# sloisel/MultiGridBarrierMPI.jl

Hardware: AMD Instinct MI355X
Metric: fem2d p-Laplace DoF/s per Newton step (higher is better)
Workload: dtype f64; 1 GPU; fem2d p-Laplace L=7 p=1 (n=57344 rows, N_L=49154 Newton unknowns), amgb main phase, tol=sqrt(eps); parallelism=single GPU

## Files before the change

include/mgb_hip.h:

```cpp
#ifndef MGB_HIP_H
#define MGB_HIP_H

#include <stdint.h>

#ifdef __cplusplus
extern "C" {
#endif

#define MGB_OK 0
#define MGB_E_ARG (-1)
#define MGB_E_HIP (-2)
#define MGB_E_NUMERIC (-3)
#define MGB_E_INTERNAL (-4)

typedef struct mgb_ctx_s* mgb_ctx;
typedef struct mgb_geo_s* mgb_geo;
typedef struct mgb_amg_s* mgb_amg;
typedef struct mgb_vec_s* mgb_vec;
typedef struct mgb_csr_s* mgb_csr;

const char* mgb_last_error(void);
int mgb_version(void);
int mgb_device_count(void);

// ... 116 lines not shown
int mgb_plan_prolongation(mgb_plan fine, mgb_plan coarse, int* rows, int* cols, int* nnz, int32_t* rowptr, int32_t* colidx,
                          double* vals);
int mgb_plan_sizes(mgb_plan p, int* N, int* nnz_lower, int* nnz_T, int* nnz_B);
int mgb_plan_pattern(mgb_plan p, int32_t* rowptr, int32_t* colidx);
int mgb_plan_eval_host(mgb_plan p, const double* Y , double* lower_vals);
int mgb_plan_shard(mgb_plan p, int S, int K, int rank, int world, int block, mgb_plan* out, int* r0, int* r1);
int mgb_plan_apply_B_host(mgb_plan p, const double* s , double* Bs );
int mgb_plan_apply_BT_host(mgb_plan p, const double* v , double* g );
int mgb_plan_chol_bench(mgb_plan p, const double* Y, int dim, int reps, double* seconds_per_factor,
                        double* seconds_per_solve, double* flops, double* front_doubles, double* residual);
typedef struct mgb_hostchol_s* mgb_hostchol;
int mgb_plan_hostchol_create(mgb_plan p, int dim, mgb_hostchol* out);
int mgb_hostchol_destroy(mgb_hostchol c);
int mgb_hostchol_info(mgb_hostchol c, int* n, int* threads, double* flops);
int mgb_hostchol_factor_solve(mgb_hostchol c, const double* lower_vals, const double* g, double* x);
int mgb_hostchol_partition(mgb_hostchol c, int world, int* split_world, int cap, int* nnodes, int* owner);
int mgb_hostchol_factor_solve_dist(mgb_hostchol c, int rank, int world, mgb_allreduce_fn fn, void* user,
                                   const double* lower_vals, const double* g, double* x);
int mgb_plan_hostchol_create_ranked(mgb_plan p, int dim, int K, int world, int block, mgb_hostchol* out);
int mgb_hostchol_rank_aligned(mgb_hostchol c, int world, int* aligned, int* top_values);
int mgb_hostchol_factor_solve_dist_local(mgb_hostchol c, int rank, int world, mgb_allreduce_fn fn, void* user,
                                         const double* local_lower_vals, const double* g, double* x);
int mgb_plan_chol_tree(mgb_plan p, int dim, int cap, int* nnodes, int* ns, int* nf, int* parent);
int mgb_chol_selftest(int nx, int ny, double* max_residual, double* flops, double* seconds);

#ifdef __cplusplus
}
#endif
#endif
```

multigridbarriermpi.jl_amd/_lib.py:

```python
from __future__ import annotations

import ctypes as C
import os

import numpy as np

_HERE = os.path.dirname(os.path.abspath(__file__))
LIB_PATH = os.path.join(_HERE, "lib", "libmgb_hip.so")

c_int_p = C.POINTER(C.c_int)
c_i32_p = C.POINTER(C.c_int32)
c_dbl_p = C.POINTER(C.c_double)
c_flt_p = C.POINTER(C.c_float)
c_ll_p = C.POINTER(C.c_longlong)
c_str_arr = C.POINTER(C.c_char_p)
H = C.c_void_p
ALLREDUCE_FN = C.CFUNCTYPE(C.c_int, C.c_void_p, C.c_void_p, C.c_longlong)


class MGBError(RuntimeError):
    def __init__(self, code, msg):
        super().__init__("mgb error %d: %s" % (code, msg))
        self.code = code

# ... 97 lines not shown
    "mgb_amg_sol_kernels": [H, c_dbl_p, c_dbl_p, c_ll_p],
    "mgb_amg_time_kernels": [H, C.c_int, C.c_int, C.c_int, c_dbl_p, c_dbl_p],
    "mgb_plan_create": [H, C.c_int, c_str_arr, C.c_int, c_str_arr, C.c_int, c_int_p, C.c_int, C.c_int,
                        C.POINTER(H)],
    "mgb_reduction_scratch_doubles": [C.c_int, C.c_int, c_ll_p],
    "mgb_plan_destroy": [H],
    "mgb_plan_sizes": [H, c_int_p, c_int_p, c_int_p, c_int_p],
    "mgb_plan_pattern": [H, c_i32_p, c_i32_p],
    "mgb_plan_eval_host": [H, c_dbl_p, c_dbl_p],
    "mgb_plan_shard": [H, C.c_int, C.c_int, C.c_int, C.c_int, C.c_int, C.POINTER(C.c_void_p), c_int_p, c_int_p],
    "mgb_plan_apply_B_host": [H, c_dbl_p, c_dbl_p],
    "mgb_plan_apply_BT_host": [H, c_dbl_p, c_dbl_p],
    "mgb_plan_chol_bench": [H, c_dbl_p, C.c_int, C.c_int, c_dbl_p, c_dbl_p, c_dbl_p, c_dbl_p, c_dbl_p],
    "mgb_plan_hostchol_create": [H, C.c_int, C.POINTER(H)],
    "mgb_hostchol_destroy": [H],
    "mgb_hostchol_info": [H, c_int_p, c_int_p, c_dbl_p],
    "mgb_hostchol_factor_solve": [H, c_dbl_p, c_dbl_p, c_dbl_p],
    "mgb_hostchol_partition": [H, C.c_int, c_int_p, C.c_int, c_int_p, c_int_p],
    "mgb_hostchol_factor_solve_dist": [H, C.c_int, C.c_int, ALLREDUCE_FN, C.c_void_p, c_dbl_p, c_dbl_p, c_dbl_p],
    "mgb_plan_hostchol_create_ranked": [H, C.c_int, C.c_int, C.c_int, C.c_int, C.POINTER(H)],
    "mgb_hostchol_rank_aligned": [H, C.c_int, c_int_p, c_int_p],
    "mgb_hostchol_factor_solve_dist_local": [H, C.c_int, C.c_int, ALLREDUCE_FN, C.c_void_p, c_dbl_p, c_dbl_p, c_dbl_p],
    "mgb_plan_chol_tree": [H, C.c_int, C.c_int, c_int_p, c_int_p, c_int_p, c_int_p],
    "mgb_chol_selftest": [C.c_int, C.c_int, c_dbl_p, c_dbl_p, c_dbl_p],
}
_SPECIAL = {"mgb_last_error": ([], C.c_char_p), "mgb_version": ([], C.c_int), "mgb_device_count": ([], C.c_int)}

_lib = None


def load():
    global _lib
    if _lib is not None:
        return _lib
    if not os.path.exists(LIB_PATH):
        raise ImportError("libmgb_hip.so not built: run `python -c 'import __graft_entry__ as g; g.build()'` "
                          "or multigridbarriermpi.jl_amd/csrc/build.sh (expected at %s)" % LIB_PATH)
    lib = C.CDLL(LIB_PATH)
    for name, args in PROTOTYPES.items():
        fn = getattr(lib, name)
        fn.argtypes = args
        fn.restype = C.c_int
    for name, (args, res) in _SPECIAL.items():
        fn = getattr(lib, name)
        fn.argtypes = args
        fn.restype = res
# ... 34 lines not shown
```

multigridbarriermpi.jl_amd/csrc/capi.cpp:

```cpp
#include "../../include/mgb_hip.h"

#include <chrono>
#include <cmath>
#include <cstdlib>
#include <string>
#include <thread>

#include "amg.hpp"

using namespace mgb;

struct mgb_ctx_s {
  Ctx ctx;
  explicit mgb_ctx_s(int dev) : ctx(dev) {}
};
struct mgb_geo_s {
  GeometryHost g;
};
struct mgb_vec_s {
  mgb_ctx_s* ctx;
  DevBuf<double> buf;
  int n;
};
struct mgb_csr_s {
// ... 1254 lines not shown
      const int rc = fn(user, ptr, count);
      if (rc != 0) throw InternalError("mgb: allreduce callback failed with code " + std::to_string(rc));
    };
    if (!c->ch.factor_solve_dist(local_lower_vals, x, part, rank, ar, true))
      throw NumericError("MfChol: matrix is not positive definite");
  });
}

int mgb_plan_chol_tree(mgb_plan p, int dim, int cap, int* nnodes, int* ns, int* nf, int* parent) {
  return guard([&] {
    need(p && nnodes, "chol_tree: bad arguments");
    MfChol ch;
    ch.analyze(p->plan.Apat, p->plan.coords.data(), dim);
    std::vector<int> a, b, c;
    ch.tree(a, b, c);
    *nnodes = (int)a.size();
    const int m = std::min<int>(cap, (int)a.size());
    if (ns) std::copy(a.begin(), a.begin() + m, ns);
    if (nf) std::copy(b.begin(), b.begin() + m, nf);
    if (parent) std::copy(c.begin(), c.begin() + m, parent);
  });
}

int mgb_chol_selftest(int nx, int ny, double* max_residual, double* flops, double* seconds) {
  return guard([&] {
    need(nx > 0 && ny > 0, "selftest: bad size");
    const int N = nx * ny;
    std::vector<Triplet> t;
    std::vector<double> coords((size_t)N * 2);
    for (int j = 0; j < ny; ++j)
      for (int i = 0; i < nx; ++i) {
        const int r = j * nx + i;
        coords[2 * r] = i;
        coords[2 * r + 1] = j;
        t.push_back({r, r, 6.0 + 1e-3 * ((r * 7919) % 13)});
        if (i > 0) t.push_back({r, r - 1, -1.0});
        if (j > 0) t.push_back({r, r - nx, -1.0});
        if (i > 0 && j > 0) t.push_back({r, r - nx - 1, -0.5});
      }
    Csr Lo = from_triplets(N, N, t);
    MfChol ch;
    ch.analyze(Lo, coords.data(), 2);
    const auto t0 = std::chrono::steady_clock::now();
    if (!ch.factor(Lo.vals.data())) throw NumericError("MfChol: selftest matrix not SPD");
    const double sec = std::chrono::duration<double>(std::chrono::steady_clock::now() - t0).count();
    std::vector<double> xs(N), b(N, 0.0);
// ... 18 lines not shown
```

multigridbarriermpi.jl_amd/csrc/gpuchol.hip:

```cpp
#include "gpuchol.hpp"

#include "amg.hpp"

#include <algorithm>
#include <array>
#include <cmath>
#include <cstdio>
#include <cstdlib>
#include <numeric>
#include <stdexcept>
#include <string>

namespace mgb {

namespace {

constexpr int PB = 32;
constexpr int LP = PB + 1;
constexpr int TS = 64;
constexpr int TB = 256;
constexpr int RT = 1024;

void ck(hipError_t e, const char* what) {
  if (e != hipSuccess) throw HipError(std::string("HIP error in gpuchol ") + what + ": " + hipGetErrorString(e));
// ... 1153 lines not shown
          for (int i = k0 + sl; i < k1; i += nsl) s = fma(F[(long long)ld * i + j], u[i], s);
        }
        if (nsl > 1) {
          red[tid] = s;
          __syncthreads();
          if (sl == 0)
            for (int q = 1; q < nsl; ++q) s += red[q * jw + jl];
        }
        if (sl == 0 && j < k0) u[j] -= s;
      }
      __syncthreads();
    }
    if (pp == npanel - 1) STAMP(5);
  }
  STAMP(6);
  for (int i = tid; i < ns; i += NT) {
    const double v = u[i];
    y[nd.first + i] = v;
    x[perm[nd.first + i]] = v;
  }
  STAMP(7);
}

__global__ __launch_bounds__(256) void schur_pack_kernel(const RootXchg* __restrict__ roots, const double* __restrict__ fronts,
                                                         double* __restrict__ xb) {
  const RootXchg r = roots[blockIdx.x];
  const double* F = fronts + r.off;
  for (int j = blockIdx.y; j < r.nb; j += gridDim.y) {
    double* dst = xb + r.xoff + (long long)j * (r.nb + 1) - (long long)j * (j - 1) / 2 - j;
    const double* col = F + (long long)r.ld * (r.ns + j) + r.ns;
    for (int i = j + threadIdx.x; i <= r.nb; i += blockDim.x) dst[i] = r.owned ? col[i] : 0.0;
  }
}

__global__ __launch_bounds__(256) void schur_unpack_kernel(const RootXchg* __restrict__ roots, const double* __restrict__ xb,
                                                           double* __restrict__ fronts) {
  const RootXchg r = roots[blockIdx.x];
  double* F = fronts + r.off;
  for (int j = blockIdx.y; j < r.nb; j += gridDim.y) {
    const double* src = xb + r.xoff + (long long)j * (r.nb + 1) - (long long)j * (j - 1) / 2 - j;
    double* col = F + (long long)r.ld * (r.ns + j) + r.ns;
    for (int i = j + threadIdx.x; i <= r.nb; i += blockDim.x) col[i] = src[i];
  }
}

__global__ __launch_bounds__(256) void vals_pack_kernel(int n, const int* __restrict__ idx, const double* __restrict__ vals,
// ... 50 lines not shown
};

const CholKnobs& GpuChol::knobs() {
  static const CholKnobs k = [] {
    auto on = [](const char* name) {
      const char* e = std::getenv(name);
      return !(e && e[0] == '0');
    };
    auto num = [](const char* name, int dflt) {
      const char* e = std::getenv(name);
      return e ? std::atoi(e) : dflt;
    };
    CholKnobs c;
    c.graph = on("MGB_CHOL_GRAPH");
    c.prof = std::getenv("MGB_CHOL_PROF") != nullptr;
    c.leaf = on("MGB_CHOL_LEAF");
    c.single = on("MGB_CHOL_SINGLE");
    c.step2 = on("MGB_CHOL_STEP2");
    c.wide = on("MGB_CHOL_WIDE");
    c.start_pivot = on("MGB_CHOL_START_PIVOT");
    c.step2_tiles = num("MGB_CHOL_STEP2_TILES", 224);
    c.dense_tiles = num("MGB_CHOL_DENSE_TILES", 512);
    c.bwd_split_nf = num("MGB_BWD_SPLIT_NF", 192);
    return c;
  }();
  return k;
}

namespace {

StepTile pivot_tile(const GNode& g, int t, int p) {
  StepTile st{};
  st.off = g.off;
  st.loff = g.loff + (long long)p * 2 * PB * PB;
  st.nf = g.nf;
  st.ns = g.ns;
  st.pad = t;
  return st;
}

int append_tiles(std::vector<StepTile>& out, const GNode& g, int t, int p, int k, bool column) {
  StepTile st = pivot_tile(g, t, p);
  const size_t n0 = out.size();
  if (column) {
    const int Tr = std::max(0, (g.nf + 1 - k - PB + TS - 1) / TS);
    for (int ti = 0; ti < Tr; ++ti) {
// ... 25 lines not shown
  u.a1 = g.a1;
  u.first = g.first;
  u.ti = s.ti;
  u.tj = s.tj;
  for (int sI = 0; sI < 2; ++sI) {
    u.boff[sI] = g.off;
    u.cld[sI] = 0;
    if (g.child[sI] >= 0) {
      const GNode& c = nodes[g.child[sI]];
      u.cld[sI] = c.nf + 1;
      u.boff[sI] = c.off + (long long)u.cld[sI] * c.ns + c.ns;
    }
  }
  return u;
}

}

int GpuChol::schedule(const std::vector<std::vector<int>>& heights, const std::vector<GNode>& nodes,
                      const std::vector<std::vector<StartJob>>& sjobs, const MfChol& sym, Jobs& jobs) {
  const CholKnobs& kn = knobs();
  std::vector<Launch> bwd;
  std::vector<StepTile> scratch;
  for (const std::vector<int>& mine : heights) {
    if (mine.empty()) continue;
    const int nofs = (int)jobs.lists.size(), ncnt = (int)mine.size();
    jobs.lists.insert(jobs.lists.end(), mine.begin(), mine.end());
    int max_ns = 0, max_nf = 0;
    bool childless = true, all_pivots = true;
    double start_bytes = 0;
    for (int t : mine) {
      const GNode& g = nodes[t];
      max_ns = std::max(max_ns, g.ns);
      max_nf = std::max(max_nf, g.nf);
      childless = childless && g.child[0] < 0 && g.child[1] < 0;
      all_pivots = all_pivots && g.ns >= 1;
      start_bytes += 0.5 * g.nf * g.nf * 8.0 + (double)sym.a_idx_[t].size() * 20.0;
      for (int c : g.child) {
        if (c < 0) continue;
        const double cnb = nodes[c].nf - nodes[c].ns;
        start_bytes += 0.5 * cnb * cnb * 8.0;
      }
    }
    const bool leaf = kn.leaf && max_nf <= 95 && max_ns <= 2 * PB && childless && all_pivots;
    const bool single = kn.single && max_ns <= PB && !childless && all_pivots;
    if (leaf) {
      const size_t lds = ((size_t)(max_nf + 1) * max_nf - (size_t)max_nf * (max_nf - 1) / 2) * sizeof(double);
// ... 68 lines not shown
      if (single) {
        const int sofs = (int)jobs.singles.size();
        for (int q = ofs; q < ofs + cnt; ++q) jobs.singles.push_back(single_tile(nodes, jobs.tiles[q]));
        const bool narrow = max_ns <= 8, dense = cnt > kn.dense_tiles;
        const Kind k = dense ? (narrow ? Kind::SingleDenseNarrow : Kind::SingleDense) : (narrow ? Kind::SingleNarrow : Kind::Single);
        chain_.push_back({k, sofs, cnt, TB, 0, 0, 0, false, KC_CHOL_SINGLE, start_bytes + bytes});
      } else {
        chain_.push_back({pair ? Kind::Step2 : Kind::Step, ofs, cnt, TB, pair ? (size_t)kStep2Lds : 0, p, npiv, false, KC_CHOL_STEP, bytes});
      }
      if (pair) ++p;
    }
    const bool split = max_nf > kn.bwd_split_nf;
    const int rofs = (int)jobs.rects.size();
    double rect_bytes = 0, tri_bytes = 0;
    for (int t : mine) {
      const GNode& g = nodes[t];
      const double nb = g.nf - g.ns;
      rect_bytes += nb * g.ns * 8.0 + nb * 12.0;
      tri_bytes += 0.5 * g.ns * g.ns * 8.0 + g.ns * 28.0;
      if (split && nb > 0)
        for (int ch = 0; ch * 64 < g.ns; ++ch) jobs.rects.push_back({t, ch});
    }
    const int nrect = (int)jobs.rects.size() - rofs, nt = max_nf > 384 ? 1024 : 256;
    std::vector<Launch> h;
    if (nrect) h.push_back({Kind::BwdRect, rofs, nrect, RT, (size_t)(max_nf + RT) * sizeof(double), 0, 0, false, KC_CHOL_BWD_RECT, rect_bytes});
    h.push_back({nt == 1024 ? Kind::Bwd1024 : Kind::Bwd256, nofs, ncnt, nt, (size_t)(max_nf + nt + PB) * sizeof(double), 0, 0, nrect > 0,
                 KC_CHOL_BWD, tri_bytes + (nrect ? 0.0 : rect_bytes)});
    bwd.insert(bwd.begin(), h.begin(), h.end());
  }
  const int first_bwd = (int)chain_.size();
  chain_.insert(chain_.end(), bwd.begin(), bwd.end());
  return first_bwd;
}

void GpuChol::build(const MfChol& sym, Ctx* ctx) {
  ctx_ = ctx;
  part_ = (ctx && ctx->world > 1) ? sym.partition(ctx->world) : CholPartition();
  if (!part_.split()) part_.owner.assign(sym.nodes_.size(), -1);
  const int my_rank = ctx ? ctx->rank : 0;
  n_ = sym.n_;
  nnodes_ = (int)sym.nodes_.size();
  flops_ = sym.flops_;
  std::vector<GNode> nodes(nnodes_);
  std::vector<int> bdry_all, ea_all, pinv, height(nnodes_, 0);
  long long off = 0, loff = 0;
  max_nf_ = 0;
  for (int t = 0; t < nnodes_; ++t) {
    const auto& nd = sym.nodes_[t];
    GNode& g = nodes[t];
    g.off = off;
    g.loff = loff;
    loff += (long long)((nd.ns + PB - 1) / PB) * 2 * PB * PB;
    g.nf = nd.nf();
    g.ns = nd.ns;
// ... 74 lines not shown
        j.a0 = (int)asrc.size();
        while (q < m && key(ord[q]) == (long long)ch * 65536 + rb) {
          const int pos = sym.a_pos_[t][ord[q]], col = pos / nf, row = pos % nf;
          if (row < col) throw InternalError("gpuchol: assembly entry above the diagonal");
          asrc.push_back(sym.a_idx_[t][ord[q]]);
          apos.push_back(ld * col + row);
          ++q;
        }
        j.a1 = (int)asrc.size();
        sjobs[t].push_back(j);
      }
    }
    if (q != m) throw InternalError("gpuchol: assembly entry outside the front");
    nodes[t].a0 = sjobs[t].empty() ? 0 : sjobs[t].front().a0;
    nodes[t].a1 = sjobs[t].empty() ? 0 : sjobs[t].back().a1;
  }
  std::vector<std::vector<int>> own(nheights_), top(nheights_);
  for (int t = 0; t < nnodes_; ++t) {
    if (!part_.split() || part_.owner[t] == my_rank) own[height[t]].push_back(t);
    else if (part_.owner[t] < 0) top[height[t]].push_back(t);
  }
  Jobs jobs;
  chain_.clear();
  own_bwd_ = schedule(own, nodes, sjobs, sym, jobs);
  top_fwd_ = (int)chain_.size();
  if (part_.split()) schedule(top, nodes, sjobs, sym, jobs);
  if ((size_t)(max_nf_ + RT + PB) * 8 > 150 * 1024) throw ArgError("gpuchol: front exceeds the LDS budget of the sweeps");
  d_nodes_ = upload(nodes);
  d_perm_ = upload(sym.perm_);
  d_bdry_ = upload(bdry_all);
  d_pinv_ = upload(pinv);
  d_asm_src_ = upload(asrc);
  d_asm_pos_ = upload(apos);
  d_lists_ = upload(jobs.lists);
  {
    std::vector<GNode> hn(jobs.lists.size()), rn(jobs.rects.size());
    for (size_t k = 0; k < jobs.lists.size(); ++k) hn[k] = nodes[jobs.lists[k]];
    for (size_t k = 0; k < jobs.rects.size(); ++k) rn[k] = nodes[jobs.rects[k].node];
    d_hnodes_ = upload(hn);
    d_rnodes_ = upload(rn);
  }
  d_start_ = upload(jobs.starts);
  d_tiles_ = upload(jobs.tiles);
  d_singles_ = upload(jobs.singles);
  d_rectjobs_ = upload(jobs.rects);
  if (part_.split()) {
    std::vector<RootXchg> roots;
    long long xoff = 0;
    for (int j = 0; j < part_.world; ++j) {
      const GNode& g = nodes[part_.roots[j]];
      RootXchg r{};
      r.off = g.off;
      r.xoff = xoff;
      r.ld = g.nf + 1;
      r.ns = g.ns;
      r.nb = g.nf - g.ns;
      r.owned = (j == my_rank) ? 1 : 0;
      xoff += (long long)r.nb * (r.nb + 3) / 2;
      max_root_nb_ = std::max(max_root_nb_, r.nb);
      roots.push_back(r);
    }
    xchg_doubles_ = xoff;
    nroots_ = (int)roots.size();
    d_roots_ = upload(roots);
    std::vector<int> own(n_, 0);
    for (int t = 0; t < nnodes_; ++t)
      if (part_.owner[t] == my_rank || (part_.owner[t] < 0 && my_rank == 0))
        for (int k = 0; k < nodes[t].ns; ++k) own[sym.perm_[nodes[t].first + k]] = 1;
// ... 32 lines not shown
  ck(hipMalloc((void**)&d_fail_, sizeof(int)), "hipMalloc flag");
  allocs_.push_back(d_fail_);
  ck(hipMemset(d_fail_, 0, sizeof(int)), "memset");
  if (knobs().prof) {
    const size_t nl = chain_.size();
    ck(hipMalloc((void**)&d_prof_, kProfSlots * nl * sizeof(long long)), "hipMalloc prof");
    allocs_.push_back(d_prof_);
    reset_stamps();
#ifdef MGB_PROF_PER_WG
    {
      long long* wg = nullptr;
      ck(hipMalloc((void**)&wg, nl * kProfMaxWg * 2 * sizeof(long long)), "hipMalloc wgprof");
      allocs_.push_back(wg);
      ck(hipMemset(wg, 0, nl * kProfMaxWg * 2 * sizeof(long long)), "memset wgprof");
      ck(hipMemcpyToSymbol(HIP_SYMBOL(g_wgprof), &wg, sizeof(wg)), "symbol wgprof");
      ck(hipMemcpyToSymbol(HIP_SYMBOL(g_prof_base), &d_prof_, sizeof(d_prof_)), "symbol prof base");
      d_wgprof_ = wg;
    }
#endif
  }
  ck(hipFuncSetAttribute((const void*)backward_kernel<256>, hipFuncAttributeMaxDynamicSharedMemorySize, 150 * 1024), "attr");
  ck(hipFuncSetAttribute((const void*)backward_kernel<1024>, hipFuncAttributeMaxDynamicSharedMemorySize, 150 * 1024), "attr");
  ck(hipFuncSetAttribute((const void*)backward_rect_kernel, hipFuncAttributeMaxDynamicSharedMemorySize, 150 * 1024), "attr");
  ck(hipFuncSetAttribute((const void*)front_leaf_kernel, hipFuncAttributeMaxDynamicSharedMemorySize, 100 * 1024), "attr");
  ck(hipFuncSetAttribute((const void*)front_step2_kernel, hipFuncAttributeMaxDynamicSharedMemorySize, kStep2Lds), "attr");
  ck(hipFuncSetAttribute((const void*)front_panel2_kernel, hipFuncAttributeMaxDynamicSharedMemorySize, kPanel2Lds), "attr");
  ck(hipFuncSetAttribute((const void*)front_update2_kernel, hipFuncAttributeMaxDynamicSharedMemorySize, kUpdate2Lds), "attr");
}

void GpuChol::factor_solve(hipStream_t st, double* d_vals, const double* d_b, double* d_x, KernelTimer* tm, bool flag_armed,
                           bool values_summed, bool x_local) {
  if (n_ == 0) return;
  if (!flag_armed) ck(hipMemsetAsync(d_fail_, 0, sizeof(int), st), "memset flag");
  if (part_.split()) {
    factor_solve_split(st, d_vals, d_b, d_x, tm, values_summed, x_local && vals_local_ && !values_summed);
    return;
  }
  if (!knobs().graph || tm || d_prof_) {
    enqueue(st, d_vals, d_b, d_x, tm);
    return;
  }
  for (const GraphEntry& g : graphs_)
    if (g.vals == d_vals && g.b == d_b && g.x == d_x) {
      ck(hipGraphLaunch(g.exec, st), "hipGraphLaunch");
      return;
    }
// ... 38 lines not shown
        break;
      case Kind::Start:
        hipLaunchKernelGGL(front_start_kernel, grid, block, L.lds, st, d_nodes_, d_start_ + L.ofs, d_pinv_, d_asm_src_, d_asm_pos_,
                           d_vals, d_perm_, d_b, d_fronts_, d_fronts_, d_linv_, d_fail_, prof, knobs().start_pivot ? 1 : 0);
        break;
      case Kind::Step:
      case Kind::Step2:
      case Kind::Panel2:
      case Kind::Update2:
        hipLaunchKernelGGL(L.kind == Kind::Step ? front_step_kernel : L.kind == Kind::Step2 ? front_step2_kernel
                           : L.kind == Kind::Panel2 ? front_panel2_kernel : front_update2_kernel,
                           grid, block, L.lds, st, d_tiles_ + L.ofs, L.p, L.npiv, d_fronts_, d_linv_, d_linv_, d_fail_, prof);
        break;
      case Kind::BwdRect:
        hipLaunchKernelGGL(backward_rect_kernel, grid, block, L.lds, st, d_rnodes_ + L.ofs, d_rectjobs_ + L.ofs, d_bdry_, d_fronts_,
                           d_y_, d_rect_);
        break;
      case Kind::Bwd256:
      case Kind::Bwd1024:
        hipLaunchKernelGGL(L.kind == Kind::Bwd1024 ? backward_kernel<1024> : backward_kernel<256>, grid, block, L.lds, st,
                           d_hnodes_ + L.ofs, d_lists_ + L.ofs, d_bdry_, d_fronts_, d_linv_, d_perm_, d_rect_, L.rect ? 1 : 0, d_y_,
                           d_x, prof);
        break;
    }
    if (tm) tm->end(st);
  }
}

void GpuChol::enqueue_chain(hipStream_t st, const double* d_vals, const double* d_b, double* d_x) {
  if (part_.split()) throw InternalError("gpuchol: a split factorisation cannot be captured");
  if (n_ == 0) return;
  run(st, 0, top_fwd_, d_vals, d_b, d_x, nullptr);
  ck(hipGetLastError(), "chain launches");
}

void GpuChol::factor_solve_split(hipStream_t st, double* d_vals, const double* d_b, double* d_x, KernelTimer* tm, bool values_summed,
                                 bool x_local) {
  const bool ride = vals_local_ && !values_summed;
  const int ntop = ride ? ntop_vals_ : 0;
  run(st, 0, own_bwd_, d_vals, d_b, d_x, tm);
  const dim3 xg(nroots_, std::max(1, std::min(64, max_root_nb_)));
  hipLaunchKernelGGL(schur_pack_kernel, xg, dim3(256), 0, st, d_roots_, d_fronts_, d_xchg_);
  const int vgrid = std::max(1, std::min(1024, (ntop_vals_ + 255) / 256));
  if (ride)
    hipLaunchKernelGGL(vals_pack_kernel, dim3(vgrid), dim3(256), 0, st, ntop_vals_, d_top_idx_, d_vals, d_xchg_ + xchg_doubles_);
  ck(hipGetLastError(), "schur pack");
// ... 91 lines not shown
```

multigridbarriermpi.jl_amd/csrc/gpuchol.hpp:

```cpp
#pragma once
#include <hip/hip_runtime.h>

#include <vector>

#include "mfchol.hpp"

namespace mgb {

class KernelTimer;
struct Ctx;

struct RootXchg {
  long long off;
  long long xoff;
  int ld, ns, nb;
  int owned;
};

struct GNode {
  long long off;
  long long loff;
  int nf, ns, first, parent;
  int bofs;
  int child[2];
  int iofs;
  int a0, a1;
};
// ... 18 lines not shown
struct SingleTile {
  long long off, loff;
  long long boff[2];
  int cld[2];
  int nf, ns, iofs, a0, a1, first;
  short ti, tj;
};

struct RectJob {
  int node, chunk;
};

struct CholKnobs {
  bool graph;
  bool prof;
  bool leaf;
  bool single;
  bool step2;
  bool wide;
  bool start_pivot;
  int step2_tiles;
  int dense_tiles;
  int bwd_split_nf;
};

class GpuChol {
 public:
  GpuChol() = default;
  GpuChol(const GpuChol&) = delete;
  GpuChol& operator=(const GpuChol&) = delete;
  ~GpuChol();
  static const CholKnobs& knobs();
  void build(const MfChol& sym, Ctx* ctx = nullptr);
  bool split() const { return part_.split(); }
  bool values_local() const { return vals_local_; }
  double exchange_doubles() const { return (double)xchg_doubles_ + ntop_vals_ + n_ + 1; }
  void factor_solve(hipStream_t st, double* d_vals, const double* d_b, double* d_x, KernelTimer* timer = nullptr,
                    bool flag_armed = false, bool values_summed = false, bool x_local = false);
  const int* unknown_kind() const { return d_kind_orig_; }
  const int* top_unknowns() const { return d_top_unk_; }
  int ntop_unknowns() const { return ntop_unk_; }
  void enqueue_chain(hipStream_t st, const double* d_vals, const double* d_b, double* d_x);
  int* fail_flag() const { return d_fail_; }
  int size() const { return n_; }
  double front_bytes() const { return (double)total_front_ * 8; }
  double factor_flops() const { return flops_; }
// ... 35 lines not shown
  int n_ = 0, nnodes_ = 0, nheights_ = 0, max_nf_ = 0;
  long long total_front_ = 0;
  double flops_ = 0;
  double* d_fronts_ = nullptr;
  double* d_rect_ = nullptr;
  double* d_linv_ = nullptr;
  double* d_y_ = nullptr;
  int* d_fail_ = nullptr;
  long long* d_prof_ = nullptr;
  [[maybe_unused]] long long* d_wgprof_ = nullptr;
  GNode* d_nodes_ = nullptr;
  int* d_perm_ = nullptr;
  int* d_bdry_ = nullptr;
  int* d_pinv_ = nullptr;
  int* d_asm_src_ = nullptr;
  int* d_asm_pos_ = nullptr;
  int* d_lists_ = nullptr;
  GNode* d_hnodes_ = nullptr;
  GNode* d_rnodes_ = nullptr;
  StartJob* d_start_ = nullptr;
  StepTile* d_tiles_ = nullptr;
  SingleTile* d_singles_ = nullptr;
  RectJob* d_rectjobs_ = nullptr;
  enum class Kind : unsigned char {
    Leaf, Single, SingleNarrow, SingleDense, SingleDenseNarrow, Start, Step, Step2, Panel2, Update2, BwdRect, Bwd256, Bwd1024
  };
  struct Launch {
    Kind kind;
    int ofs, cnt;
    int block;
    size_t lds;
    int p, npiv;
    bool rect;
    int timer;
    double bytes;
  };
  std::vector<Launch> chain_;
  int own_bwd_ = 0, top_fwd_ = 0;
  std::vector<void*> allocs_;
};

}
```

multigridbarriermpi.jl_amd/csrc/mfchol.hpp:

```cpp
#pragma once
#include <atomic>
#include <functional>
#include <vector>

#include "sparse.hpp"

namespace mgb {

struct CholPartition {
  int world = 1;
  std::vector<int> owner;
  std::vector<int> roots;
  bool split() const { return world > 1; }
};

class MfChol {
 public:
  void analyze(const Csr& pattern, const double* coords, int dim, int leaf_size = 64, const unsigned long long* rank_mask = nullptr,
               int world = 1);
  bool factor(const double* vals);
  void solve(double* b) const;
  typedef std::function<void(double*, long long)> Allreduce;
  bool factor_solve_dist(const double* vals, double* b, const CholPartition& part, int rank, const Allreduce& allreduce,
                         bool vals_local = false);
  bool rank_aligned(int world) const { return world > 1 && aligned_world_ == world; }
  std::vector<int> top_value_indices(const CholPartition& part) const;
  CholPartition partition(int world) const;
  int size() const { return n_; }
  static int threads();
  size_t front_doubles() const { return fronts_total_; }
  double factor_flops() const { return flops_; }
  int num_nodes() const { return (int)nodes_.size(); }
  int max_front() const { return max_front_; }
  void tree(std::vector<int>& ns, std::vector<int>& nf, std::vector<int>& parent) const {
    ns.clear(); nf.clear(); parent.clear();
    for (const Node& nd : nodes_) { ns.push_back(nd.ns); nf.push_back(nd.nf()); parent.push_back(nd.parent); }
  }

 private:
  friend class GpuChol;
  struct Node {
    int parent = -1;
    int first = 0, ns = 0;
    std::vector<int> bdry;
    std::vector<int> children;
    std::vector<int> ea;
    size_t off = 0;
    int nf() const { return ns + (int)bdry.size(); }
  };
  struct Subtree {
    std::vector<Node> nodes;
    std::vector<std::vector<int>> own;
  };
  int build(std::vector<int>& dofs, int lo, int hi, const Csr& A, const double* coords, int dim, int leaf,
            std::vector<int>& label, std::atomic<int>& next_label, Subtree& sub, int par_depth,
            const unsigned long long* mask = nullptr, int rlo = 0, int rhi = 1);
  void factor_node(int t, const double* vals, bool& ok);
  void forward_node(int t, double* y) const;
  void backward_node(int t, double* y) const;
  int n_ = 0, max_front_ = 0, aligned_world_ = 1, a_nnz_ = 0;
// ... 13 lines not shown
```

Measured before the change: 83.90 million DoF/s per Newton step.

## Add fused single-kernel backward sweep over lower elimination-tree subtrees

Adds a planner and a HIP kernel that run the supernodal Cholesky backward solve for the lower levels of the elimination tree in a single launch. Each workgroup handles one subtree plus its ancestor chain, staging slot maps and solution entries in LDS. This replaces the per-height BwdRect/Bwd launches for those levels, aiming to cut launch overhead and global-memory round trips. It is gated behind an environment knob and brings substantial complexity, LDS pressure and some redundant ancestor work per workgroup.

```diff
diff --git a/include/mgb_hip.h b/include/mgb_hip.h
--- a/include/mgb_hip.h
+++ b/include/mgb_hip.h
@@ -162,6 +162,8 @@
 int mgb_hostchol_factor_solve_dist_local(mgb_hostchol c, int rank, int world, mgb_allreduce_fn fn, void* user,
                                          const double* local_lower_vals, const double* g, double* x);
 int mgb_plan_chol_tree(mgb_plan p, int dim, int cap, int* nnodes, int* ns, int* nf, int* parent);
+int mgb_plan_chol_bwd_fused(mgb_plan p, int dim, int cut, int top_nf, int threads, int* info, int cap_wg, int* wg, int cap_bdry,
+                            int* bdry, int* slots, int cap_nodes, int* bofs, int* first);
 int mgb_chol_selftest(int nx, int ny, double* max_residual, double* flops, double* seconds);
 
 #ifdef __cplusplus
diff --git a/multigridbarriermpi.jl_amd/_lib.py b/multigridbarriermpi.jl_amd/_lib.py
--- a/multigridbarriermpi.jl_amd/_lib.py
+++ b/multigridbarriermpi.jl_amd/_lib.py
@@ -143,6 +143,8 @@
     "mgb_hostchol_rank_aligned": [H, C.c_int, c_int_p, c_int_p],
     "mgb_hostchol_factor_solve_dist_local": [H, C.c_int, C.c_int, ALLREDUCE_FN, C.c_void_p, c_dbl_p, c_dbl_p, c_dbl_p],
     "mgb_plan_chol_tree": [H, C.c_int, C.c_int, c_int_p, c_int_p, c_int_p, c_int_p],
+    "mgb_plan_chol_bwd_fused": [H, C.c_int, C.c_int, C.c_int, C.c_int, c_int_p, C.c_int, c_int_p, C.c_int, c_int_p, c_int_p, C.c_int,
+                                c_int_p, c_int_p],
     "mgb_chol_selftest": [C.c_int, C.c_int, c_dbl_p, c_dbl_p, c_dbl_p],
 }
 _SPECIAL = {"mgb_last_error": ([], C.c_char_p), "mgb_version": ([], C.c_int), "mgb_device_count": ([], C.c_int)}
diff --git a/multigridbarriermpi.jl_amd/csrc/bwd_fused.cpp b/multigridbarriermpi.jl_amd/csrc/bwd_fused.cpp
--- /dev/null
+++ b/multigridbarriermpi.jl_amd/csrc/bwd_fused.cpp
@@ -0,0 +1,211 @@
+#include "bwd_fused.hpp"
+
+#include <algorithm>
+
+#include "errors.hpp"
+
+namespace mgb {
+
+namespace {
+constexpr int PB = 32;
+int round64(int v) { return (v + 63) & ~63; }
+}
+
+FusedPlan plan_bwd_fused(const std::vector<int>& ns, const std::vector<int>& first, const std::vector<int>& parent,
+                         const std::vector<const std::vector<int>*>& bdry, const FusedKnobs& kn) {
+  FusedPlan P;
+  const int n = (int)ns.size();
+  if (kn.threads < 64 || kn.threads > 512 || (kn.threads & (kn.threads - 1))) throw ArgError("gpuchol: fused backward sweep: bad thread count");
+  P.threads = kn.threads;
+  P.height.assign(n, 0);
+  P.bofs.assign(n, 0);
+  std::vector<long long> off(n), loff(n);
+  std::vector<int> nf(n);
+  {
+    long long o = 0, lo = 0;
+    int b = 0;
+    for (int t = 0; t < n; ++t) {
+      nf[t] = ns[t] + (int)bdry[t]->size();
+      off[t] = o;
+      loff[t] = lo;
+      P.bofs[t] = b;
+      o += (long long)(nf[t] + 1) * (nf[t] + 1);
+      lo += (long long)((ns[t] + PB - 1) / PB) * 2 * PB * PB;
+      b += (int)bdry[t]->size();
+      if (parent[t] >= 0) {
+        if (parent[t] <= t) throw InternalError("gpuchol: elimination tree is not in postorder");
+        P.height[parent[t]] = std::max(P.height[parent[t]], P.height[t] + 1);
+      }
+    }
+    P.slots.assign(b, -1);
+  }
+  if (n == 0) return P;
+  P.nheights = *std::max_element(P.height.begin(), P.height.end()) + 1;
+  std::vector<int> hmax(P.nheights, 0);
+  for (int t = 0; t < n; ++t) hmax[P.height[t]] = std::max(hmax[P.height[t]], nf[t]);
+  int h_top = -1;
+  while (h_top + 1 < P.nheights && (kn.top_nf <= 0 || hmax[h_top + 1] <= kn.top_nf)) ++h_top;
+  if (h_top < 0) return P;
+  int h_cut = std::min(std::max(kn.cut, 0), h_top);
+  auto count_roots = [&](int c) {
+    int k = 0;
+    for (int t = 0; t < n; ++t) k += P.height[t] <= c && (parent[t] < 0 || P.height[parent[t]] > c);
+    return k;
+  };
+  if (kn.max_wg > 0) {
+    for (int raised = 0; raised < kn.max_raise && h_cut < h_top && count_roots(h_cut) > kn.max_wg; ++raised) ++h_cut;
+    if (count_roots(h_cut) > kn.max_wg) return P;
+  }
+  std::vector<int> roots, root_of(n, -1), minfirst(first);
+  for (int t = 0; t < n; ++t)
+    if (parent[t] >= 0) minfirst[parent[t]] = std::min(minfirst[parent[t]], minfirst[t]);
+  for (int t = n - 1; t >= 0; --t) {
+    if (P.height[t] > h_cut) continue;
+    if (parent[t] >= 0 && P.height[parent[t]] <= h_cut) root_of[t] = root_of[parent[t]];
+    else root_of[t] = t;
+  }
+  for (int t = 0; t < n; ++t)
+    if (root_of[t] == t) roots.push_back(t);
+  std::vector<int> above(n, 0), base(n, 0);
+  for (int t = n - 1; t >= 0; --t)
+    if (parent[t] >= 0) above[t] = above[parent[t]] + ns[parent[t]];
+  for (int t = 0; t < n; ++t) {
+    const int r = root_of[t];
+    if (r < 0) {
+      base[t] = above[t];
+      continue;
+    }
+    if (first[r] + ns[r] - minfirst[r] < 0 || first[t] < minfirst[r] || first[t] + ns[t] > first[r] + ns[r])
+      throw InternalError("gpuchol: subtree unknowns are not contiguous");
+    base[t] = above[r] + first[t] - minfirst[r];
+  }
+  for (int t = 0; t < n; ++t) {
+    if (P.height[t] > h_top) continue;
+    const std::vector<int>& bd = *bdry[t];
+    int a = parent[t];
+    for (size_t i = 0; i < bd.size(); ++i) {
+      while (a >= 0 && !(bd[i] >= first[a] && bd[i] < first[a] + ns[a])) a = parent[a];
+      if (a < 0) {
+        a = parent[t];
+        while (a >= 0 && !(bd[i] >= first[a] && bd[i] < first[a] + ns[a])) a = parent[a];
+        if (a < 0) throw InternalError("gpuchol: boundary entry outside the ancestors");
+      }
+      const int ab = (root_of[a] >= 0) ? base[a] : above[a];
+      P.slots[P.bofs[t] + i] = ab + bd[i] - first[a];
+    }
+  }
+  auto nsl_rect = [&](int t) {
+    const int h = P.height[t], nb = nf[t] - ns[t];
+    if (nb == 0 || ns[t] == 0) return 0;
+    if (hmax[h] > kn.split_nf) return 1024 / 64;
+    const int nt = hmax[h] > 384 ? 1024 : 256;
+    return nt / std::min(nt, round64(ns[t]));
+  };
+  const int W = kn.threads / 64;
+  struct Rec {
+    std::vector<std::vector<int>> levels;
+    int first_solve = 0, sub_level = 0;
+  };
+  std::vector<Rec> recs(roots.size());
+  std::vector<char> stored(n, 0);
+  std::vector<std::vector<int>> kids(n);
+  for (int t = 0; t < n; ++t)
+    if (parent[t] >= 0) kids[parent[t]].push_back(t);
+  size_t max_jobs = 0;
+  for (size_t w = 0; w < roots.size(); ++w) {
+    Rec& R = recs[w];
+    const int r = roots[w];
+    std::vector<int> anc;
+    for (int a = parent[r]; a >= 0; a = parent[a]) anc.push_back(a);
+    std::reverse(anc.begin(), anc.end());
+    std::vector<int> ab;
+    for (int a : anc)
+      if (P.height[a] > h_top) ab.push_back(a);
+    if (!ab.empty()) {
+      R.levels.push_back(ab);
+      R.first_solve = 1;
+    }
+    for (int a : anc)
+      if (P.height[a] <= h_top) R.levels.push_back({a});
+    R.sub_level = (int)R.levels.size();
+    std::vector<int> cur{r};
+    while (!cur.empty()) {
+      R.levels.push_back(cur);
+      std::vector<int> nxt;
+      for (int t : cur) nxt.insert(nxt.end(), kids[t].begin(), kids[t].end());
+      cur.swap(nxt);
+    }
+    size_t nj = 0;
+    for (const auto& l : R.levels) nj += l.size();
+    max_jobs = std::max(max_jobs, nj);
+    P.max_levels = std::max(P.max_levels, (int)R.levels.size());
+  }
+  P.h_top = h_top;
+  P.h_cut = h_cut;
+  P.nwg = (int)roots.size();
+  const int jo = kFusedHdr + kFusedLevelInts * P.max_levels;
+  P.wstride = jo + kFusedJobInts * (int)max_jobs;
+  P.wg.assign((size_t)P.nwg * P.wstride, 0);
+  for (size_t w = 0; w < roots.size(); ++w) {
+    const Rec& R = recs[w];
+    int* rec = P.wg.data() + w * P.wstride;
+    const int r = roots[w];
+    int nj = 0, sl = 0;
+    for (size_t l = 0; l < R.levels.size(); ++l) {
+      const std::vector<int>& lv = R.levels[l];
+      int* li = rec + kFusedHdr + kFusedLevelInts * l;
+      const bool solve = (int)l >= R.first_solve;
+      int maxp = 0, items = 0;
+      li[0] = nj;
+      li[1] = (int)lv.size();
+      for (int t : lv) {
+        int* j = rec + jo + kFusedJobInts * nj++;
+        const int nsl = solve ? nsl_rect(t) : 0;
+        int flags = 0;
+        if (!solve) flags = 2;
+        else if (root_of[t] >= 0 || !stored[t]) {
+          flags = 1;
+          stored[t] = 1;
+        }
+        j[FJ_OFF] = (int)(off[t] & 0xffffffffLL);
+        j[FJ_OFF + 1] = (int)(off[t] >> 32);
+        j[FJ_LOFF] = (int)(loff[t] & 0xffffffffLL);
+        j[FJ_LOFF + 1] = (int)(loff[t] >> 32);
+        j[FJ_FIRST] = first[t];
+        j[FJ_NF] = nf[t];
+        j[FJ_NS] = ns[t];
+        j[FJ_SOFS] = P.bofs[t];
+        j[FJ_BASE] = base[t];
+        j[FJ_LSOFS] = sl;
+        j[FJ_NSL] = nsl;
+        j[FJ_NT] = hmax[P.height[t]] > 384 ? 1024 : 256;
+        j[FJ_FLAGS] = flags;
+        j[FJ_NODE] = t;
+        if (solve) {
+          sl += nf[t] - ns[t];
+          maxp = std::max(maxp, (ns[t] + PB - 1) / PB);
+          items = std::max(items, nsl * ns[t]);
+        }
+      }
+      li[2] = maxp;
+      li[3] = items;
+      if (solve) {
+        int G = W;
+        while (G > 1 && W / G < (int)lv.size()) G >>= 1;
+        P.red_cap = std::max(P.red_cap, (W / G) * items);
+      }
+    }
+    rec[0] = (int)R.levels.size();
+    rec[1] = nj;
+    rec[2] = R.first_solve;
+    rec[3] = above[r] + first[r] + ns[r] - minfirst[r];
+    rec[4] = sl;
+    rec[5] = R.sub_level;
+    P.xs_cap = std::max(P.xs_cap, rec[3]);
+    P.sl_cap = std::max(P.sl_cap, sl);
+  }
+  P.lds_bytes = (size_t)P.wstride * 4 + (size_t)(P.xs_cap + P.red_cap) * 8 + (size_t)P.sl_cap * 4;
+  return P;
+}
+
+}
diff --git a/multigridbarriermpi.jl_amd/csrc/bwd_fused.hpp b/multigridbarriermpi.jl_amd/csrc/bwd_fused.hpp
--- /dev/null
+++ b/multigridbarriermpi.jl_amd/csrc/bwd_fused.hpp
@@ -0,0 +1,51 @@
+#pragma once
+#include <cstddef>
+#include <vector>
+
+namespace mgb {
+
+struct FusedKnobs {
+  int cut = 2;
+  int max_wg = 256;
+  int max_raise = 2;
+  int top_nf = 384;
+  int threads = 512;
+  int split_nf = 192;
+};
+
+constexpr int kFusedHdr = 8;
+constexpr int kFusedLevelInts = 4;
+constexpr int kFusedJobInts = 16;
+enum FusedJobField {
+  FJ_OFF = 0,
+  FJ_LOFF = 2,
+  FJ_FIRST = 4,
+  FJ_NF = 5,
+  FJ_NS = 6,
+  FJ_SOFS = 7,
+  FJ_BASE = 8,
+  FJ_LSOFS = 9,
+  FJ_NSL = 10,
+  FJ_NT = 11,
+  FJ_FLAGS = 12,
+  FJ_NODE = 13
+};
+
+struct FusedPlan {
+  int h_top = -1, h_cut = -1, nwg = 0, nheights = 0;
+  int wstride = 0;
+  int max_levels = 0;
+  int xs_cap = 0, sl_cap = 0, red_cap = 0;
+  int threads = 0;
+  size_t lds_bytes = 0;
+  std::vector<int> wg;
+  std::vector<int> slots;
+  std::vector<int> bofs;
+  std::vector<int> height;
+  bool enabled() const { return nwg > 0; }
+};
+
+FusedPlan plan_bwd_fused(const std::vector<int>& ns, const std::vector<int>& first, const std::vector<int>& parent,
+                         const std::vector<const std::vector<int>*>& bdry, const FusedKnobs& kn);
+
+}
diff --git a/multigridbarriermpi.jl_amd/csrc/capi.cpp b/multigridbarriermpi.jl_amd/csrc/capi.cpp
--- a/multigridbarriermpi.jl_amd/csrc/capi.cpp
+++ b/multigridbarriermpi.jl_amd/csrc/capi.cpp
@@ -1300,6 +1300,34 @@
   });
 }
 
+int mgb_plan_chol_bwd_fused(mgb_plan p, int dim, int cut, int top_nf, int threads, int* info, int cap_wg, int* wg, int cap_bdry,
+                            int* bdry, int* slots, int cap_nodes, int* bofs, int* first) {
+  return guard([&] {
+    need(p && info, "chol_bwd_fused: bad arguments");
+    MfChol ch;
+    ch.analyze(p->plan.Apat, p->plan.coords.data(), dim);
+    std::vector<int> ns, fi, par, bd;
+    std::vector<const std::vector<int>*> lists;
+    ch.bwd_tables(ns, fi, par, lists);
+    FusedKnobs kn;
+    kn.cut = cut;
+    kn.top_nf = top_nf;
+    kn.threads = threads;
+    kn.split_nf = GpuChol::knobs().bwd_split_nf;
+    const FusedPlan P = plan_bwd_fused(ns, fi, par, lists, kn);
+    for (const std::vector<int>* l : lists) bd.insert(bd.end(), l->begin(), l->end());
+    const int v[12] = {P.h_top, P.h_cut, P.nwg, P.wstride, P.max_levels, P.xs_cap, P.red_cap, P.sl_cap, (int)P.lds_bytes,
+                       (int)bd.size(), (int)ns.size(), P.nheights};
+    std::copy(v, v + 12, info);
+    if (wg) std::copy(P.wg.begin(), P.wg.begin() + std::min<size_t>(cap_wg, P.wg.size()), wg);
+    const size_t mb = std::min<size_t>(cap_bdry, bd.size()), mn = std::min<size_t>(cap_nodes, ns.size());
+    if (bdry) std::copy(bd.begin(), bd.begin() + mb, bdry);
+    if (slots) std::copy(P.slots.begin(), P.slots.begin() + mb, slots);
+    if (bofs) std::copy(P.bofs.begin(), P.bofs.begin() + mn, bofs);
+    if (first) std::copy(fi.begin(), fi.begin() + mn, first);
+  });
+}
+
 int mgb_chol_selftest(int nx, int ny, double* max_residual, double* flops, double* seconds) {
   return guard([&] {
     need(nx > 0 && ny > 0, "selftest: bad size");
diff --git a/multigridbarriermpi.jl_amd/csrc/gpuchol.hip b/multigridbarriermpi.jl_amd/csrc/gpuchol.hip
--- a/multigridbarriermpi.jl_amd/csrc/gpuchol.hip
+++ b/multigridbarriermpi.jl_amd/csrc/gpuchol.hip
@@ -1199,6 +1199,214 @@
   STAMP(7);
 }
 
+
+__device__ __forceinline__ void load_pivot_block(double (&lc)[PB], const double* __restrict__ lpp, int lane) {
+#pragma unroll
+  for (int m = 0; m < PB; ++m) lc[m] = lpp[PB * m + (lane & 31)];
+}
+
+__device__ __forceinline__ void load_panel_rows(double (&f)[PB], const double* __restrict__ F, int ld, int k0, int kw, int jc) {
+  const double* Fj = F + (long long)ld * k0 + max(min(jc, k0 - 1), 0);
+#pragma unroll
+  for (int r = 0; r < PB; ++r) f[r] = Fj[(long long)ld * min(r, kw - 1)];
+}
+
+__device__ __forceinline__ void panel_substitute(const double (&lc)[PB], double* up, int kw, int lane) {
+  const int c = lane & 31;
+  double uc = (c < kw) ? up[c] : 0.0;
+#pragma unroll
+  for (int m = PB - 1; m >= 0; --m) {
+    const double xm = readlane_f64(uc * lc[m], m);
+    uc = (c == m) ? xm : fma(-lc[m], xm, uc);
+  }
+  if (lane < kw) up[c] = uc;
+}
+
+template <int NSL>
+__device__ __forceinline__ double panel_dot(const double (&f)[PB], const double* up, int kw) {
+  double s[NSL];
+#pragma unroll
+  for (int q = 0; q < NSL; ++q) s[q] = 0.0;
+#pragma unroll
+  for (int r = 0; r < PB; ++r) {
+    const double v = fma(f[r], up[min(r, kw - 1)], s[r % NSL]);
+    s[r % NSL] = (r < kw) ? v : s[r % NSL];
+  }
+  double t = s[0];
+#pragma unroll
+  for (int q = 1; q < NSL; ++q) t += s[q];
+  return t;
+}
+
+__device__ inline double panel_dot_any(const double* __restrict__ Fj, long long ld, const double* up, int kw, int nsl) {
+  double t = 0.0;
+  for (int q = 0; q < nsl; ++q) {
+    double s = 0.0;
+    for (int r = q; r < kw; r += nsl) s = fma(Fj[ld * r], up[r], s);
+    t = q ? t + s : s;
+  }
+  return t;
+}
+
+__device__ __forceinline__ int uni(int v) { return __builtin_amdgcn_readfirstlane(v); }
+
+__global__ __launch_bounds__(512) void backward_fused_kernel(const int* __restrict__ wgs, int wstride, int max_levels, int xs_cap,
+                                                              int red_cap, const int* __restrict__ slots,
+                                                              const double* __restrict__ fronts, const double* __restrict__ linv,
+                                                              const int* __restrict__ perm, double* y, double* x, long long* prof) {
+  extern __shared__ double sh[];
+  STAMP(0);
+  int* rec = (int*)sh;
+  double* xs = sh + wstride / 2;
+  double* red = xs + xs_cap;
+  int* sl = (int*)(red + red_cap);
+  const int tid = threadIdx.x, T = blockDim.x, W = T >> 6, wave = uni(tid >> 6), lane = tid & 63;
+  {
+    const int* src = wgs + (size_t)blockIdx.x * wstride;
+    for (int i = tid; i < wstride; i += T) rec[i] = src[i];
+  }
+  __syncthreads();
+  const int nlevels = rec[0], njobs = rec[1], first_lv = rec[2], sub_lv = rec[5];
+  const int* jobs = rec + kFusedHdr + kFusedLevelInts * max_levels;
+  for (int jb = wave; jb < njobs; jb += W) {
+    const int* j = jobs + kFusedJobInts * jb;
+    const int nf = uni(j[FJ_NF]), ns = uni(j[FJ_NS]), flags = uni(j[FJ_FLAGS]), base = uni(j[FJ_BASE]);
+    const long long off = ((long long)uni(j[FJ_OFF + 1]) << 32) | (unsigned)uni(j[FJ_OFF]);
+    const double* srcv = (flags & 2) ? y + uni(j[FJ_FIRST]) : fronts + off + (long long)(nf + 1) * nf;
+    for (int i0 = 0; i0 < ns; i0 += 256) {
+      double v[4];
+#pragma unroll
+      for (int k = 0; k < 4; ++k) {
+        const int i = i0 + 64 * k + lane;
+        v[k] = srcv[min(i, ns - 1)];
+      }
+#pragma unroll
+      for (int k = 0; k < 4; ++k) {
+        const int i = i0 + 64 * k + lane;
+        if (i < ns) xs[base + i] = v[k];
+      }
+    }
+    if (flags & 2) continue;
+    const int nb = nf - ns;
+    const int* ssrc = slots + uni(j[FJ_SOFS]);
+    int* sdst = sl + uni(j[FJ_LSOFS]);
+    for (int i0 = 0; i0 < nb; i0 += 256) {
+      int v[4];
+#pragma unroll
+      for (int k = 0; k < 4; ++k) {
+        const int i = i0 + 64 * k + lane;
+        v[k] = ssrc[min(i, nb - 1)];
+      }
+#pragma unroll
+      for (int k = 0; k < 4; ++k) {
+        const int i = i0 + 64 * k + lane;
+        if (i < nb) sdst[i] = v[k];
+      }
+    }
+  }
+  __syncthreads();
+  STAMP(1);
+  if (first_lv == sub_lv) STAMP(2);
+  for (int lv = first_lv; lv < nlevels; ++lv) {
+    const int* li = rec + kFusedHdr + kFusedLevelInts * lv;
+    const int lofs = li[0], cnt = li[1], maxp = li[2], items = li[3];
+    int G = W;
+    while (G > 1 && W / G < cnt) G >>= 1;
+    const int ngrp = W / G, GT = G << 6, grp = wave / G, gtid = tid - grp * GT, gw = wave - grp * G;
+    double* redg = red + grp * items;
+    for (int r0 = 0; r0 < cnt; r0 += ngrp) {
+      const bool act = r0 + grp < cnt;
+      const int* j = jobs + kFusedJobInts * (lofs + (act ? r0 + grp : 0));
+      const int nf = uni(j[FJ_NF]), ns = uni(j[FJ_NS]), nsl = uni(j[FJ_NSL]), nt = uni(j[FJ_NT]), nb = nf - ns, ld = nf + 1;
+      const long long off = ((long long)uni(j[FJ_OFF + 1]) << 32) | (unsigned)uni(j[FJ_OFF]);
+      const long long loff = ((long long)uni(j[FJ_LOFF + 1]) << 32) | (unsigned)uni(j[FJ_LOFF]);
+      const double* F = fronts + off;
+      double* u = xs + uni(j[FJ_BASE]);
+      const int npanel = (ns + PB - 1) / PB;
+      const bool sub = act && gw == 0 && npanel > 0;
+      double lc[PB], f[PB];
+      if (sub) load_pivot_block(lc, linv + loff + (long long)(npanel - 1) * 2 * PB * PB, lane);
+      if (items > 0) {
+        if (act && nsl > 0) {
+          const int* sj = sl + uni(j[FJ_LSOFS]);
+          const int nit = ns * nsl, R = (nb + nsl - 1) / nsl;
+          for (int it0 = gtid; it0 < nit; it0 += 2 * GT) {
+            const int it1 = it0 + GT;
+            const bool has1 = it1 < nit;
+            const int q0 = it0 / ns, q1 = has1 ? it1 / ns : q0;
+            const double* c0 = F + (long long)ld * ns + (it0 - q0 * ns);
+            const double* c1 = F + (long long)ld * ns + (has1 ? it1 - q1 * ns : it0 - q0 * ns);
+            double s0 = 0.0, s1 = 0.0;
+            for (int r0 = 0; r0 < R; r0 += 8) {
+              double a0[8], a1[8];
+#pragma unroll
+              for (int k = 0; k < 8; ++k) {
+                a0[k] = c0[(long long)ld * min(q0 + (r0 + k) * nsl, nb - 1)];
+                a1[k] = c1[(long long)ld * min(q1 + (r0 + k) * nsl, nb - 1)];
+              }
+#pragma unroll
+              for (int k = 0; k < 8; ++k) {
+                const int i0 = q0 + (r0 + k) * nsl, i1 = q1 + (r0 + k) * nsl;
+                const double v0 = fma(a0[k], xs[sj[min(i0, nb - 1)]], s0), v1 = fma(a1[k], xs[sj[min(i1, nb - 1)]], s1);
+                s0 = (i0 < nb) ? v0 : s0;
+                s1 = (i1 < nb) ? v1 : s1;
+              }
+            }
+            redg[it0] = s0;
+            if (has1) redg[it1] = s1;
+          }
+        }
+        __syncthreads();
+        if (act && nsl > 0)
+          for (int jc = gtid; jc < ns; jc += GT) {
+            double s = redg[jc];
+            for (int q = 1; q < nsl; ++q) s += redg[q * ns + jc];
+            u[jc] = u[jc] - s;
+          }
+        __syncthreads();
+      }
+      if (act && npanel > 1) load_panel_rows(f, F, ld, (npanel - 1) * PB, ns - (npanel - 1) * PB, gtid);
+      for (int it = 0; it < maxp; ++it) {
+        const int pp = npanel - 1 - it, k0 = pp * PB, kw = min(PB, ns - k0);
+        if (sub && pp >= 0) {
+          panel_substitute(lc, u + k0, kw, lane);
+          if (pp > 0) load_pivot_block(lc, linv + loff + (long long)(pp - 1) * 2 * PB * PB, lane);
+        }
+        __syncthreads();
+        if (it == maxp - 1) break;
+        if (act && pp > 0) {
+          const int jw = min(nt, (k0 + 63) & ~63), nslp = nt / jw;
+          for (int jc = gtid; jc < k0; jc += GT) {
+            double s;
+            if (jc >= GT) {
+              s = panel_dot_any(F + (long long)ld * k0 + jc, ld, u + k0, kw, nslp);
+            } else if (nslp == 1 || nslp == 2 || nslp == 4) {
+              s = nslp == 1 ? panel_dot<1>(f, u + k0, kw) : nslp == 2 ? panel_dot<2>(f, u + k0, kw) : panel_dot<4>(f, u + k0, kw);
+            } else {
+              s = panel_dot_any(F + (long long)ld * k0 + jc, ld, u + k0, kw, nslp);
+            }
+            u[jc] -= s;
+          }
+          if (pp > 1) load_panel_rows(f, F, ld, k0 - PB, PB, gtid);
+        }
+        __syncthreads();
+      }
+      if (act && (uni(j[FJ_FLAGS]) & 1)) {
+        const int first = uni(j[FJ_FIRST]);
+        for (int i = gtid; i < ns; i += GT) {
+          const double v = u[i];
+          y[first + i] = v;
+          x[perm[first + i]] = v;
+        }
+      }
+    }
+    if (lv + 1 == sub_lv) STAMP(2);
+    if (lv >= sub_lv) STAMP(min(3 + lv - sub_lv, 6));
+  }
+  for (int k = 3 + nlevels - sub_lv; k < 7; ++k) STAMP(k);
+  STAMP(7);
+}
+
 __global__ __launch_bounds__(256) void schur_pack_kernel(const RootXchg* __restrict__ roots, const double* __restrict__ fronts,
                                                          double* __restrict__ xb) {
   const RootXchg r = roots[blockIdx.x];
@@ -1295,6 +1503,10 @@
     c.step2_tiles = num("MGB_CHOL_STEP2_TILES", 224);
     c.dense_tiles = num("MGB_CHOL_DENSE_TILES", 512);
     c.bwd_split_nf = num("MGB_BWD_SPLIT_NF", 192);
+    c.bwd_fused = on("MGB_CHOL_BWD_FUSED");
+    c.bwd_cut = num("MGB_CHOL_BWD_CUT", 2);
+    c.bwd_fused_nf = num("MGB_CHOL_BWD_FUSED_NF", 384);
+    c.bwd_fused_threads = num("MGB_CHOL_BWD_FUSED_THREADS", 512);
     return c;
   }();
   return k;
@@ -1366,7 +1578,10 @@
   const CholKnobs& kn = knobs();
   std::vector<Launch> bwd;
   std::vector<StepTile> scratch;
-  for (const std::vector<int>& mine : heights) {
+  const bool fused = fused_.enabled() && &heights == fused_heights_;
+  double fused_bytes = 0;
+  for (size_t hh = 0; hh < heights.size(); ++hh) {
+    const std::vector<int>& mine = heights[hh];
     if (mine.empty()) continue;
     const int nofs = (int)jobs.lists.size(), ncnt = (int)mine.size();
     jobs.lists.insert(jobs.lists.end(), mine.begin(), mine.end());
@@ -1481,6 +1696,11 @@
         for (int ch = 0; ch * 64 < g.ns; ++ch) jobs.rects.push_back({t, ch});
     }
     const int nrect = (int)jobs.rects.size() - rofs, nt = max_nf > 384 ? 1024 : 256;
+    if (fused && (int)hh <= fused_.h_top) {
+      jobs.rects.resize(rofs);
+      fused_bytes += rect_bytes + tri_bytes;
+      continue;
+    }
     std::vector<Launch> h;
     if (nrect) h.push_back({Kind::BwdRect, rofs, nrect, RT, (size_t)(max_nf + RT) * sizeof(double), 0, 0, false, KC_CHOL_BWD_RECT, rect_bytes});
     h.push_back({nt == 1024 ? Kind::Bwd1024 : Kind::Bwd256, nofs, ncnt, nt, (size_t)(max_nf + nt + PB) * sizeof(double), 0, 0, nrect > 0,
@@ -1489,6 +1709,8 @@
   }
   const int first_bwd = (int)chain_.size();
   chain_.insert(chain_.end(), bwd.begin(), bwd.end());
+  if (fused)
+    chain_.push_back({Kind::BwdFused, 0, fused_.nwg, fused_.threads, fused_.lds_bytes, 0, 0, false, KC_CHOL_BWD, fused_bytes});
   return first_bwd;
 }
 
@@ -1609,7 +1831,33 @@
   }
   Jobs jobs;
   chain_.clear();
+  fused_ = FusedPlan();
+  fused_heights_ = nullptr;
+  if (!part_.split() && knobs().bwd_fused) {
+    std::vector<int> ns(nnodes_), first(nnodes_), parent(nnodes_);
+    std::vector<const std::vector<int>*> bd(nnodes_);
+    for (int t = 0; t < nnodes_; ++t) {
+      ns[t] = nodes[t].ns;
+      first[t] = nodes[t].first;
+      parent[t] = nodes[t].parent;
+      bd[t] = &sym.nodes_[t].bdry;
+    }
+    const CholKnobs& kn = knobs();
+    FusedKnobs fk;
+    fk.cut = kn.bwd_cut;
+    fk.top_nf = kn.bwd_fused_nf;
+    fk.threads = kn.bwd_fused_threads;
+    fk.split_nf = kn.bwd_split_nf;
+    fused_ = plan_bwd_fused(ns, first, parent, bd, fk);
+    if (fused_.lds_bytes > 150 * 1024) fused_ = FusedPlan();
+    if (fused_.enabled()) {
+      fused_heights_ = &own;
+      for (int t = 0; t < nnodes_; ++t)
+        if (fused_.bofs[t] != nodes[t].bofs || fused_.height[t] != height[t]) throw InternalError("gpuchol: fused plan disagrees with the front layout");
+    }
+  }
   own_bwd_ = schedule(own, nodes, sjobs, sym, jobs);
+  fused_heights_ = nullptr;
   top_fwd_ = (int)chain_.size();
   if (part_.split()) schedule(top, nodes, sjobs, sym, jobs);
   if ((size_t)(max_nf_ + RT + PB) * 8 > 150 * 1024) throw ArgError("gpuchol: front exceeds the LDS budget of the sweeps");
@@ -1631,6 +1879,8 @@
   d_tiles_ = upload(jobs.tiles);
   d_singles_ = upload(jobs.singles);
   d_rectjobs_ = upload(jobs.rects);
+  d_fused_wg_ = upload(fused_.wg);
+  d_fused_slots_ = upload(fused_.slots);
   if (part_.split()) {
     std::vector<RootXchg> roots;
     long long xoff = 0;
@@ -1709,6 +1959,7 @@
   ck(hipFuncSetAttribute((const void*)backward_kernel<256>, hipFuncAttributeMaxDynamicSharedMemorySize, 150 * 1024), "attr");
   ck(hipFuncSetAttribute((const void*)backward_kernel<1024>, hipFuncAttributeMaxDynamicSharedMemorySize, 150 * 1024), "attr");
   ck(hipFuncSetAttribute((const void*)backward_rect_kernel, hipFuncAttributeMaxDynamicSharedMemorySize, 150 * 1024), "attr");
+  ck(hipFuncSetAttribute((const void*)backward_fused_kernel, hipFuncAttributeMaxDynamicSharedMemorySize, 150 * 1024), "attr");
   ck(hipFuncSetAttribute((const void*)front_leaf_kernel, hipFuncAttributeMaxDynamicSharedMemorySize, 100 * 1024), "attr");
   ck(hipFuncSetAttribute((const void*)front_step2_kernel, hipFuncAttributeMaxDynamicSharedMemorySize, kStep2Lds), "attr");
   ck(hipFuncSetAttribute((const void*)front_panel2_kernel, hipFuncAttributeMaxDynamicSharedMemorySize, kPanel2Lds), "attr");
@@ -1793,6 +2044,10 @@
                            d_hnodes_ + L.ofs, d_lists_ + L.ofs, d_bdry_, d_fronts_, d_linv_, d_perm_, d_rect_, L.rect ? 1 : 0, d_y_,
                            d_x, prof);
         break;
+      case Kind::BwdFused:
+        hipLaunchKernelGGL(backward_fused_kernel, grid, block, L.lds, st, d_fused_wg_, fused_.wstride, fused_.max_levels,
+                           fused_.xs_cap, fused_.red_cap, d_fused_slots_, d_fronts_, d_linv_, d_perm_, d_y_, d_x, prof);
+        break;
     }
     if (tm) tm->end(st);
   }
diff --git a/multigridbarriermpi.jl_amd/csrc/gpuchol.hpp b/multigridbarriermpi.jl_amd/csrc/gpuchol.hpp
--- a/multigridbarriermpi.jl_amd/csrc/gpuchol.hpp
+++ b/multigridbarriermpi.jl_amd/csrc/gpuchol.hpp
@@ -3,6 +3,7 @@
 
 #include <vector>
 
+#include "bwd_fused.hpp"
 #include "mfchol.hpp"
 
 namespace mgb {
@@ -67,6 +68,10 @@
   int step2_tiles;
   int dense_tiles;
   int bwd_split_nf;
+  bool bwd_fused;
+  int bwd_cut;
+  int bwd_fused_nf;
+  int bwd_fused_threads;
 };
 
 class GpuChol {
@@ -148,8 +153,12 @@
   StepTile* d_tiles_ = nullptr;
   SingleTile* d_singles_ = nullptr;
   RectJob* d_rectjobs_ = nullptr;
+  const std::vector<std::vector<int>>* fused_heights_ = nullptr;
+  FusedPlan fused_;
+  int* d_fused_wg_ = nullptr;
+  int* d_fused_slots_ = nullptr;
   enum class Kind : unsigned char {
-    Leaf, Single, SingleNarrow, SingleDense, SingleDenseNarrow, Start, Step, Step2, Panel2, Update2, BwdRect, Bwd256, Bwd1024
+    Leaf, Single, SingleNarrow, SingleDense, SingleDenseNarrow, Start, Step, Step2, Panel2, Update2, BwdRect, Bwd256, Bwd1024, BwdFused
   };
   struct Launch {
     Kind kind;
diff --git a/multigridbarriermpi.jl_amd/csrc/mfchol.hpp b/multigridbarriermpi.jl_amd/csrc/mfchol.hpp
--- a/multigridbarriermpi.jl_amd/csrc/mfchol.hpp
+++ b/multigridbarriermpi.jl_amd/csrc/mfchol.hpp
@@ -36,6 +36,10 @@
     ns.clear(); nf.clear(); parent.clear();
     for (const Node& nd : nodes_) { ns.push_back(nd.ns); nf.push_back(nd.nf()); parent.push_back(nd.parent); }
   }
+  void bwd_tables(std::vector<int>& ns, std::vector<int>& first, std::vector<int>& parent, std::vector<const std::vector<int>*>& bdry) const {
+    ns.clear(); first.clear(); parent.clear(); bdry.clear();
+    for (const Node& nd : nodes_) { ns.push_back(nd.ns); first.push_back(nd.first); parent.push_back(nd.parent); bdry.push_back(&nd.bdry); }
+  }
 
  private:
   friend class GpuChol;
```

Measured after the change: 88.42 million DoF/s per Newton step (median of 6 runs). 5.4% higher.
